# kobby-pentangeli/chaum-pedersen-zkp

Hardware: AMD Instinct MI355X
Metric: verified proofs/sec (1/2/4/8 MI355X) + % int-VALU roofline vs host-CPU (higher is better)
Workload: dtype int32/int64 limbs (GF(2^255-19), radix 2^25.5)

## Files before the change

### chaum-pedersen-zkp_amd/build_native.py

```python
from __future__ import annotations

import os
import shutil
import subprocess
import sys
from concurrent.futures import ThreadPoolExecutor

PKG = os.path.dirname(os.path.abspath(__file__))
ROOT = os.path.dirname(PKG)
CSRC = os.path.join(PKG, "csrc")
LIBDIR = os.path.join(PKG, "lib")
LIBCPZ = os.path.join(LIBDIR, "libcpz.so")
HOSTTEST = os.path.join(ROOT, "tests", "native", "libcpz_hosttest.so")
DEVPROBE = os.path.join(ROOT, "tests", "native", "libcpz_devprobe.so")
PARTPROBE = os.path.join(ROOT, "tests", "native", "libcpz_partprobe.so")
PARTPAIRSPROBE = os.path.join(ROOT, "tests", "native", "libcpz_partpairsprobe.so")
MSMPROBE = os.path.join(ROOT, "tests", "native", "libcpz_msmprobe.so")
PAIRSUMPROBE = os.path.join(ROOT, "tests", "native", "libcpz_pairsumprobe.so")
PREPPROBE = os.path.join(ROOT, "tests", "native", "libcpz_prepprobe.so")
MICROPROBE = os.path.join(ROOT, "tests", "native", "libcpz_microprobe.so")
ARCH = os.environ.get("CPZ_OFFLOAD_ARCH", "gfx950")


def _hipcc() -> str:
    for cand in (shutil.which("hipcc"), "/opt/rocm/bin/hipcc"):
        if cand and os.path.exists(cand):
            return cand
    raise RuntimeError("hipcc not found: the gfx950 build needs ROCm")


def _newer(out: str, srcs) -> bool:
    if not os.path.exists(out):
        return True
    t = os.path.getmtime(out)
    return any(os.path.getmtime(s) > t for s in srcs)


def _headers():
    hdr = [os.path.join(CSRC, f) for f in os.listdir(CSRC) if f.endswith(".h")]
    return hdr + [os.path.join(ROOT, "include", "cpz.h")]


def _run(cmd):
    r = subprocess.run(cmd, stdout=subprocess.PIPE, stderr=subprocess.STDOUT, text=True)
    if r.returncode != 0:
        raise RuntimeError("build step failed: %s\n%s" % (" ".join(cmd), r.stdout[-4000:]))
    return r.stdout


UNIT_FLAGS = {"wide.hip": ["-falign-loops=64"]}


def build_libcpz(force: bool = False, verbose: bool = False, out: str = LIBCPZ, defines=()) -> str:
    units = ["kernels.hip", "wide.hip", "rlc.hip", "part.hip", "runtime.hip"]
    srcs = [os.path.join(CSRC, u) for u in units] + _headers()
    if not force and not defines and not _newer(out, srcs):
        return out
    objdir = os.path.join(os.path.dirname(out), "obj" if not defines else "obj_" + "_".join(defines).replace("=", ""))
    os.makedirs(objdir, exist_ok=True)
    hipcc = _hipcc()
    common = [hipcc, "--offload-arch=" + ARCH, "-O3", "-std=c++17", "-fPIC", "-I", CSRC,
              "-I", os.path.join(ROOT, "include")] + ["-D" + d for d in defines]
    if defines and os.environ.get("CPZ_EXTRA_FLAGS"):
        common += os.environ["CPZ_EXTRA_FLAGS"].split()

    def compile_one(u):
        obj = os.path.join(objdir, u.replace(".hip", ".o"))
        if force or defines or _newer(obj, [os.path.join(CSRC, u)] + _headers()):
            uf = [] if defines and os.environ.get("CPZ_NO_UNIT_FLAGS") else UNIT_FLAGS.get(u, [])
            _run(common + uf + ["-c", os.path.join(CSRC, u), "-o", obj])
        return obj

    with ThreadPoolExecutor(max_workers=len(units)) as ex:
        objs = list(ex.map(compile_one, units))
    tmp = out + ".tmp"
    _run([hipcc, "--offload-arch=" + ARCH, "-shared", "-fPIC", "-o", tmp] + objs)
    os.replace(tmp, out)
    if verbose:
        print("built", out)
    return out


CLOCK_PROBE_LIB = os.path.join(LIBDIR, "timing", "clock_probe.so")


def build_clock_probe(force: bool = False) -> str:
    os.makedirs(os.path.dirname(CLOCK_PROBE_LIB), exist_ok=True)
    return build_libcpz(force, out=CLOCK_PROBE_LIB, defines=("CPZ_CLOCK_PROBE", "CPZ_TIMING_ONLY"))


def build_hosttest(force: bool = False, out: str = HOSTTEST, defines=()) -> str:
    srcs = [os.path.join(ROOT, "tests", "native", f) for f in ("hostlib.cpp", "hostlib_joint.cpp", "hostlib_lean.cpp",
                                                              "hostlib_prove.cpp", "hostlib_pairsum.cpp")]
    if not force and not _newer(out, srcs + _headers()):
        return out
    cxx = shutil.which("g++") or "g++"
    tmp = out + ".tmp"
    extra = ["-D" + d for d in os.environ.get("CPZ_HOST_DEFINES", "").split() + list(defines)]
    _run([cxx, "-O2", "-std=c++17", "-fPIC", "-shared", "-DCPZ_BOUNDS_CHECK", "-DCPZ_COUNT_OPS"] + extra +
         ["-I", CSRC] + srcs + ["-o", tmp])
    os.replace(tmp, out)
    return out


def build_devprobe(force: bool = False, out: str = DEVPROBE, include: str = CSRC) -> str:
    src = os.path.join(ROOT, "tests", "native", "devprobe.hip")
    hdrs = [os.path.join(include, f) for f in os.listdir(include) if f.endswith(".h")]
    if not force and not _newer(out, [src] + hdrs):
        return out
    tmp = out + ".tmp"
    _run([_hipcc(), "--offload-arch=" + ARCH, "-O3", "-std=c++17", "-fPIC", "-I", include,
          "-I", os.path.join(ROOT, "include"), "-shared", src, "-o", tmp])
    os.replace(tmp, out)
    return out


def build_partprobe(force: bool = False, out: str = PARTPROBE, include: str = CSRC) -> str:
    src = os.path.join(ROOT, "tests", "native", "partprobe.hip")
    deps = [os.path.join(include, f) for f in os.listdir(include) if f.endswith(".h") or f == "part.hip"]
    if not force and not _newer(out, [src] + deps):
        return out
    tmp = out + ".tmp"
    _run([_hipcc(), "--offload-arch=" + ARCH, "-O3", "-std=c++17", "-fPIC", "-I", include,
          "-I", os.path.join(ROOT, "include"), "-shared", src, "-o", tmp])
    os.replace(tmp, out)
    return out


def build_partpairsprobe(force: bool = False, out: str = PARTPAIRSPROBE, include: str = CSRC) -> str:
    src = os.path.join(ROOT, "tests", "native", "partpairsprobe.hip")
    deps = [os.path.join(include, f) for f in os.listdir(include) if f.endswith(".h") or f == "part.hip"]
    if not force and not _newer(out, [src] + deps):
        return out
    tmp = out + ".tmp"
    _run([_hipcc(), "--offload-arch=" + ARCH, "-O3", "-std=c++17", "-fPIC", "-I", include,
          "-I", os.path.join(ROOT, "include"), "-shared", src, "-o", tmp])
    os.replace(tmp, out)
    return out


def build_msmprobe(force: bool = False, out: str = MSMPROBE, include: str = CSRC) -> str:
    src = os.path.join(ROOT, "tests", "native", "msmprobe.hip")
    deps = [os.path.join(include, f) for f in os.listdir(include) if f.endswith(".h") or f == "rlc.hip"]
    if not force and not _newer(out, [src] + deps):
        return out
    tmp = out + ".tmp"
    _run([_hipcc(), "--offload-arch=" + ARCH, "-O3", "-std=c++17", "-fPIC", "-I", include,
          "-I", os.path.join(ROOT, "include"), "-shared", src, "-o", tmp])
    os.replace(tmp, out)
    return out


def build_pairsumprobe(force: bool = False, out: str = PAIRSUMPROBE, include: str = CSRC) -> str:
    src = os.path.join(ROOT, "tests", "native", "pairsumprobe.hip")
    deps = [os.path.join(include, f) for f in os.listdir(include) if f.endswith(".h") or f == "rlc.hip"]
    if not force and not _newer(out, [src] + deps):
        return out
    tmp = out + ".tmp"
    _run([_hipcc(), "--offload-arch=" + ARCH, "-O3", "-std=c++17", "-fPIC", "-I", include,
          "-I", os.path.join(ROOT, "include"), "-shared", src, "-o", tmp])
    os.replace(tmp, out)
    return out


def build_prepprobe(force: bool = False, out: str = PREPPROBE, include: str = CSRC) -> str:
    src = os.path.join(ROOT, "tests", "native", "prepprobe.hip")
    deps = [os.path.join(include, f) for f in os.listdir(include) if f.endswith(".h") or f == "rlc.hip"]
    if not force and not _newer(out, [src] + deps):
        return out
    tmp = out + ".tmp"
    _run([_hipcc(), "--offload-arch=" + ARCH, "-O3", "-std=c++17", "-fPIC", "-I", include,
          "-I", os.path.join(ROOT, "include"), "-shared", src, "-o", tmp])
    os.replace(tmp, out)
    return out


# ... 82 lines not shown
```

### chaum-pedersen-zkp_amd/csrc/fe25519.h

```cpp
#pragma once
#include <stdint.h>

#if defined(__HIPCC__)
#define CPZ_HD __host__ __device__ __forceinline__
#define CPZ_HDM __host__ __device__ __forceinline__
#else
#define CPZ_HD static inline
#define CPZ_HDM inline
#endif


#if defined(CPZ_BOUNDS_CHECK) && !defined(__HIP_DEVICE_COMPILE__)
#include <stdio.h>
#include <stdlib.h>
#define CPZ_ASSERT(c)                                                        \
  do {                                                                       \
    if (!(c)) {                                                              \
      fprintf(stderr, "cpz bound violated %s:%d: %s\n", __FILE__, __LINE__, #c); \
      abort();                                                               \
    }                                                                        \
  } while (0)
#else
#define CPZ_ASSERT(c) ((void)0)
#endif

namespace cpz {

#if defined(CPZ_COUNT_OPS) && !defined(__HIP_DEVICE_COMPILE__)
struct OpCounts {
  unsigned long long mul, sq;
};
inline OpCounts& op_counts() {
  static thread_local OpCounts c{0, 0};
  return c;
}
#define CPZ_COUNT(field) (++::cpz::op_counts().field)
#else
#define CPZ_COUNT(field) ((void)0)
#endif

struct fe {
  int32_t v[10];
};

constexpr int32_t kLooseBound = 108000000;

CPZ_HD fe fe_const(int32_t a0, int32_t a1, int32_t a2, int32_t a3, int32_t a4, int32_t a5,
                   int32_t a6, int32_t a7, int32_t a8, int32_t a9) {
  fe r;
  r.v[0] = a0; r.v[1] = a1; r.v[2] = a2; r.v[3] = a3; r.v[4] = a4;
  r.v[5] = a5; r.v[6] = a6; r.v[7] = a7; r.v[8] = a8; r.v[9] = a9;
  return r;
}

CPZ_HD fe fe_zero() { return fe_const(0, 0, 0, 0, 0, 0, 0, 0, 0, 0); }
CPZ_HD fe fe_one() { return fe_const(1, 0, 0, 0, 0, 0, 0, 0, 0, 0); }

CPZ_HD fe FE_D() { return fe_const(56195235, 13857412, 51736253, 6949390, 114729, 24766616, 60832955, 30306712, 48412415, 21499315); }
CPZ_HD fe FE_D2() { return fe_const(45281625, 27714825, 36363642, 13898781, 229458, 15978800, 54557047, 27058993, 29715967, 9444199); }
CPZ_HD fe FE_SQRT_M1() { return fe_const(34513072, 25610706, 9377949, 3500415, 12389472, 33281959, 41962654, 31548777, 326685, 11406482); }
CPZ_HD fe FE_INVSQRT_A_MINUS_D() { return fe_const(6111466, 4156064, 39310137, 12243467, 41204824, 120896, 20826367, 26493656, 6093567, 31568420); }
CPZ_HD fe FE_SQRT_AD_MINUS_ONE() { return fe_const(24849947, 33400850, 43495378, 6347714, 46036536, 32887293, 41837720, 18186727, 66238516, 14525638); }
CPZ_HD fe FE_ONE_MINUS_D_SQ() { return fe_const(6275446, 16937061, 44170319, 29780721, 11667076, 7397348, 39186143, 1766194, 42675006, 672202); }
CPZ_HD fe FE_INV2() { return fe_const(10, 0, 0, 0, 0, 0, 0, 0, 0, -16777216); }
CPZ_HD fe FE_D_MINUS_ONE_SQ() { return fe_const(15551776, 22456977, 53683765, 23429360, 55212328, 10178283, 40474537, 4729243, 61826754, 23438029); }

CPZ_HD fe fe_add(const fe& a, const fe& b) {
  fe r;
#pragma unroll
  for (int i = 0; i < 10; i++) r.v[i] = a.v[i] + b.v[i];
  return r;
}

CPZ_HD fe fe_sub(const fe& a, const fe& b) {
  fe r;
#pragma unroll
  for (int i = 0; i < 10; i++) r.v[i] = a.v[i] - b.v[i];
  return r;
}

CPZ_HD fe fe_neg(const fe& a) {
  fe r;
#pragma unroll
  for (int i = 0; i < 10; i++) r.v[i] = -a.v[i];
  return r;
}

CPZ_HD fe fe_select(const fe& a, const fe& b, bool c) {
  fe r;
#pragma unroll
  for (int i = 0; i < 10; i++) r.v[i] = c ? b.v[i] : a.v[i];
  return r;
}

#if defined(CPZ_BOUNDS_CHECK) && !defined(__HIP_DEVICE_COMPILE__)
CPZ_HD void fe_check_operand(const fe& a) {
  for (int i = 0; i < 10; i++) CPZ_ASSERT(a.v[i] < kLooseBound && a.v[i] > -kLooseBound);
}
#else
CPZ_HD void fe_check_operand(const fe&) {}
#endif

CPZ_HD constexpr int64_t carry_bias(int k) { return (k & 1) ? (1LL << 24) : (1LL << 25); }

CPZ_HD int64_t acc_pin(int64_t x) {
#if defined(__HIP_DEVICE_COMPILE__)
  asm("" : "+v"(x));
#endif
  return x;
}

CPZ_HD int32_t opaque_sgpr(int32_t x) {
#if defined(__HIP_DEVICE_COMPILE__)
  asm("" : "+s"(x));
#endif
  return x;
}

CPZ_HD int32_t unbias_limb(int64_t H, int k) {
  const uint32_t mask = (k & 1) ? 0x1ffffffu : 0x3ffffffu;
  return (int32_t)(((uint32_t)H & mask) - (uint32_t)carry_bias(k));
}

CPZ_HD fe fe_carry_biased(int64_t H[10]) {
  fe r;
  uint32_t small = 0;
#pragma unroll
  for (int k = 0; k < 9; k++) {
    const int w = (k & 1) ? 25 : 26;
    const int32_t hi = (int32_t)(H[k] >> 32);
    const uint32_t lo = (uint32_t)H[k];
    H[k + 1] = acc_pin((int64_t)hi * (int64_t)opaque_sgpr(1 << (32 - w)) + H[k + 1]);
    r.v[k] = (int32_t)((lo & ((1u << w) - 1u)) - (uint32_t)carry_bias(k) + small);
    small = lo >> w;
  }
  const int32_t hi9 = (int32_t)(H[9] >> 32);
  const uint32_t lo9 = (uint32_t)H[9];
  r.v[9] = (int32_t)((lo9 & 0x1ffffffu) - (uint32_t)carry_bias(9) + small);
  const int64_t h0 = (int64_t)hi9 * (int64_t)opaque_sgpr(19 << 7) +
                     (int64_t)(uint64_t)(((uint32_t)r.v[0] + (uint32_t)carry_bias(0)) + 19u * (lo9 >> 25));
  r.v[1] += (int32_t)(h0 >> 26);
  r.v[0] = unbias_limb(h0, 0);
  return r;
}

CPZ_HD fe fe_carry_wide(int64_t h[10]) {
#pragma unroll
  for (int k = 0; k < 10; k++) h[k] += carry_bias(k);
  return fe_carry_biased(h);
}

CPZ_HD fe fe_mul(const fe& f, const fe& g) {
  CPZ_COUNT(mul);
  fe_check_operand(f);
  fe_check_operand(g);
  int32_t g19[10], f2[10];
#pragma unroll
  for (int i = 0; i < 10; i++) {
    g19[i] = (int32_t)(19u * (uint32_t)g.v[i]);
    f2[i] = (int32_t)(2u * (uint32_t)f.v[i]);
  }
  int64_t h[10];
#pragma unroll
  for (int i = 0; i < 10; i++) {
#pragma unroll
    for (int k = 0; k < 10; k++) {
      const int j = (k - i + 10) % 10;
      const int32_t a = ((i & 1) && (j & 1)) ? f2[i] : f.v[i];
      const int32_t b = (i + j >= 10) ? g19[j] : g.v[j];
      h[k] = acc_pin((int64_t)a * (int64_t)b + (i == 0 ? carry_bias(k) : h[k]));
    }
  }
  fe r = fe_carry_biased(h);
  return r;
}

CPZ_HD void fe_sq_wide(int64_t h[10], const fe& f, int div) {
  CPZ_COUNT(sq);
  fe_check_operand(f);
  int32_t f2[10], f19[10];
#pragma unroll
  for (int i = 0; i < 10; i++) {
    f2[i] = (int32_t)(2u * (uint32_t)f.v[i]);
    f19[i] = (int32_t)(19u * (uint32_t)f.v[i]);
  }
  bool first[10] = {true, true, true, true, true, true, true, true, true, true};
#pragma unroll
  for (int i = 0; i < 10; i++) {
#pragma unroll
    for (int j = i; j < 10; j++) {
      const int k = (i + j) % 10;
      const int m2 = (i != j ? 2 : 1) * (((i & 1) && (j & 1)) ? 2 : 1);
      const int32_t a = (m2 == 1) ? f.v[i] : (m2 == 2 ? f2[i] : (int32_t)(2u * (uint32_t)f2[i]));
      const int32_t b = (i + j >= 10) ? f19[j] : f.v[j];
      h[k] = acc_pin((int64_t)a * (int64_t)b + (first[k] ? (div ? carry_bias(k) / div : 0) : h[k]));
      first[k] = false;
    }
  }
}

CPZ_HD fe fe_sq(const fe& f) {
  int64_t h[10];
  fe_sq_wide(h, f, 1);
  fe r = fe_carry_biased(h);
  return r;
}

CPZ_HD fe fe_sq2(const fe& f) {
  int64_t h[10];
  fe_sq_wide(h, f, 2);
#pragma unroll
  for (int i = 0; i < 10; i++) h[i] += h[i];
  fe r = fe_carry_biased(h);
  return r;
}

CPZ_HD fe fe_carry_floor(int64_t H[10]) {
  fe r;
#pragma unroll
  for (int k = 0; k < 9; k++) {
    H[k + 1] += H[k] >> ((k & 1) ? 25 : 26);
    r.v[k] = (int32_t)((uint32_t)H[k] & ((k & 1) ? 0x1ffffffu : 0x3ffffffu));
  }
  const int64_t h0 = (int64_t)r.v[0] + 19 * (H[9] >> 25);
  r.v[9] = (int32_t)((uint32_t)H[9] & 0x1ffffffu);
  r.v[1] += (int32_t)(h0 >> 26);
  r.v[0] = (int32_t)((uint32_t)h0 & 0x3ffffffu);
  return r;
}

CPZ_HD fe fe_sqn(fe f, int n) {
#pragma unroll 1
  for (int i = 1; i < n; i++) {
    int64_t h[10];
    fe_sq_wide(h, f, 0);
    f = fe_carry_floor(h);
  }
  return fe_sq(f);
}

CPZ_HD void fe_tobytes(uint8_t s[32], const fe& f) {
  int64_t h[10];
#pragma unroll
  for (int i = 0; i < 10; i++) h[i] = f.v[i];
  fe t = fe_carry_wide(h);
#pragma unroll
  for (int i = 0; i < 10; i++) h[i] = t.v[i];
  int64_t q = (19 * h[9] + (1 << 24)) >> 25;
  q = (h[0] + q) >> 26;
  q = (h[1] + q) >> 25;
  q = (h[2] + q) >> 26;
  q = (h[3] + q) >> 25;
  q = (h[4] + q) >> 26;
  q = (h[5] + q) >> 25;
  q = (h[6] + q) >> 26;
  q = (h[7] + q) >> 25;
  q = (h[8] + q) >> 26;
  q = (h[9] + q) >> 25;
  h[0] += 19 * q;
  int64_t c;
  c = h[0] >> 26; h[1] += c; h[0] -= c * (1LL << 26);
  c = h[1] >> 25; h[2] += c; h[1] -= c * (1LL << 25);
  c = h[2] >> 26; h[3] += c; h[2] -= c * (1LL << 26);
  c = h[3] >> 25; h[4] += c; h[3] -= c * (1LL << 25);
  c = h[4] >> 26; h[5] += c; h[4] -= c * (1LL << 26);
  c = h[5] >> 25; h[6] += c; h[5] -= c * (1LL << 25);
  c = h[6] >> 26; h[7] += c; h[6] -= c * (1LL << 26);
  c = h[7] >> 25; h[8] += c; h[7] -= c * (1LL << 25);
  c = h[8] >> 26; h[9] += c; h[8] -= c * (1LL << 26);
  c = h[9] >> 25; h[9] -= c * (1LL << 25);
  uint32_t w[8];
  const uint32_t l0 = (uint32_t)h[0], l1 = (uint32_t)h[1], l2 = (uint32_t)h[2], l3 = (uint32_t)h[3],
                 l4 = (uint32_t)h[4], l5 = (uint32_t)h[5], l6 = (uint32_t)h[6], l7 = (uint32_t)h[7],
                 l8 = (uint32_t)h[8], l9 = (uint32_t)h[9];
  w[0] = l0 | (l1 << 26);
  w[1] = (l1 >> 6) | (l2 << 19);
  w[2] = (l2 >> 13) | (l3 << 13);
  w[3] = (l3 >> 19) | (l4 << 6);
  w[4] = l5 | (l6 << 25);
  w[5] = (l6 >> 7) | (l7 << 19);
  w[6] = (l7 >> 13) | (l8 << 12);
  w[7] = (l8 >> 20) | (l9 << 6);
#pragma unroll
  for (int i = 0; i < 8; i++) {
    s[4 * i + 0] = (uint8_t)(w[i]);
    s[4 * i + 1] = (uint8_t)(w[i] >> 8);
    s[4 * i + 2] = (uint8_t)(w[i] >> 16);
    s[4 * i + 3] = (uint8_t)(w[i] >> 24);
  }
}

CPZ_HD void fe_towords(uint32_t w[8], const fe& f) {
  uint8_t s[32];
  fe_tobytes(s, f);
#pragma unroll
  for (int i = 0; i < 8; i++)
    w[i] = (uint32_t)s[4 * i] | ((uint32_t)s[4 * i + 1] << 8) | ((uint32_t)s[4 * i + 2] << 16) |
// ... 124 lines not shown
```

### chaum-pedersen-zkp_amd/csrc/kernels.hip

```cpp
#include <hip/hip_runtime.h>

#include <cstddef>
#include <type_traits>

#include "cpz_kernels.h"
#include "ristretto.h"
#include "scalar25519.h"
#include "transcript.h"
#include "scalarmul.h"
#include "verify.h"
#include "rlc_dev.h"
#include "fe16.h"
#include "keccak_wave.h"
#include "proof_digits.h"

namespace cpz {

__device__ __forceinline__ bool words_zero(const uint32_t w[8]) {
  uint32_t acc = 0;
#pragma unroll
  for (int k = 0; k < 8; k++) acc |= w[k];
  return acc == 0;
}

// ... 254 lines not shown
    if ((j >> bit) & 1) acc = ge_add(acc, Q);
  }
  comb[t] = p3_to_niels(acc);
}

__device__ __forceinline__ uint32_t be32_at(const uint8_t* p) {
  return ((uint32_t)p[0] << 24) | ((uint32_t)p[1] << 16) | ((uint32_t)p[2] << 8) | (uint32_t)p[3];
}

__device__ __forceinline__ void words_at(uint32_t w[8], const uint8_t* p) {
#pragma unroll
  for (int k = 0; k < 8; k++)
    w[k] = (uint32_t)p[4 * k] | ((uint32_t)p[4 * k + 1] << 8) | ((uint32_t)p[4 * k + 2] << 16) |
           ((uint32_t)p[4 * k + 3] << 24);
}

__global__ void __launch_bounds__(256) k_parse_proofs(ParseArgs a) {
  const int64_t i = (int64_t)blockIdx.x * 256 + threadIdx.x;
  if (i >= a.n) return;
  const uint64_t o0 = a.off[i];
  const uint64_t len = a.off[i + 1] - o0;
  const uint8_t* b = a.blob + o0;
  uint32_t f0[8], f1[8], f2[8];
#pragma unroll
  for (int k = 0; k < 8; k++) f0[k] = f1[k] = f2[k] = 0;
  uint8_t code = kParseOk;
  uint32_t aux = 0;
  if (len < 1 + 4 + 1 + 4 + 1 + 4 + 1) {
    code = kParseTooSmall;
    aux = (uint32_t)len;
  } else if (b[0] != 1) {
    code = kParseBadVersion;
    aux = b[0];
  } else {
    uint64_t pos = 1;
#pragma unroll 1
    for (int q = 0; q < 3 && code == kParseOk; q++) {
      const uint8_t base = (uint8_t)(kParseR1LenMissing + 5 * q);
      const uint32_t maxlen = q < 2 ? 4096u : 512u;
      if (pos + 4 > len) { code = base; break; }
      const uint32_t fl = be32_at(b + pos);
      pos += 4;
      if (fl == 0 || fl > maxlen) { code = base + 1; aux = fl; break; }
      if (pos + fl > len) { code = base + 2; break; }
      if (fl != 32) { code = base + 3; aux = fl; break; }
      uint32_t w[8];
      words_at(w, b + pos);
      pos += 32;
      bool ok;
      if (q < 2) {
        ge_p3 P;
        ok = ristretto_decode(P, w);
      } else {
        ok = sc_is_canonical(w);
      }
      if (!ok) { code = base + 4; break; }
#pragma unroll
      for (int k = 0; k < 8; k++) {
        f0[k] = q == 0 ? w[k] : f0[k];
        f1[k] = q == 1 ? w[k] : f1[k];
        f2[k] = q == 2 ? w[k] : f2[k];
      }
    }
    if (code == kParseOk && pos != len) {
      code = kParseTrailing;
      aux = (uint32_t)(len - pos);
    }
    if (code == kParseOk) {
      if (words_zero(f0) || words_zero(f1)) code = kParseIdentity;
      else if (words_zero(f2)) code = kParseZeroS;
    }
  }
  store_words8(a.r1, i, f0);
  store_words8(a.r2, i, f1);
  store_words8(a.s, i, f2);
  a.code[i] = code;
  if (a.aux) a.aux[i] = aux;
}


#ifndef CPZ_VERIFY_WAVES
#define CPZ_VERIFY_WAVES 2
#endif
__device__ __forceinline__ void verify_one_row(const VerifyArgs& a, int64_t i, const CombTable& comb_g,
                                               const CombTable& comb_h, const SlabTable& tab, uint32_t* dig,
                                               uint32_t* rows) {
  const uint32_t* src[4] = {a.y1, a.y2, a.r1, a.r2};
  uint32_t sw[8], cw[8];
#pragma unroll
  for (int q = 0; q < 4; q++) {
    uint32_t w[8];
    load_words8(w, src[q], i);
#pragma unroll
    for (int k = 0; k < 8; k++) rows[(8 * q + k) * kVerifyBlock] = w[k];
  }
  load_words8(sw, a.s, i);
  load_words8(cw, a.c, i);
  const uint8_t st_s = a.status[i];
  const DigitRef y1{rows, kVerifyBlock}, y2{rows + 8 * kVerifyBlock, kVerifyBlock},
      r1{rows + 16 * kVerifyBlock, kVerifyBlock}, r2{rows + 24 * kVerifyBlock, kVerifyBlock};
  a.status[i] = verify_proof(y1, y2, r1, r2, sw, cw, st_s, comb_g, comb_h, tab, dig, kVerifyBlock, nullptr,
                             a.eq_only != 0);
}

__global__ void __launch_bounds__(kVerifyBlock, CPZ_VERIFY_WAVES) k_verify_prepared(VerifyArgs a) {
  const CombTable comb_g{a.comb}, comb_h{a.comb + kCombPerBase};
  const int64_t l = (int64_t)blockIdx.x * kVerifyBlock + threadIdx.x;
  int64_t i = l;
  if (a.blocks) {
    const int64_t lb = (int64_t)blockIdx.x * (kVerifyBlock / a.block_proofs) + threadIdx.x / a.block_proofs;
    if (lb >= a.nblocks) return;
    i = (int64_t)a.blocks[lb] * a.block_proofs + threadIdx.x % a.block_proofs;
  }
  if (i >= a.n) return;
  const SlabTable tab{a.scratch, (uint32_t)l * (uint32_t)(kCachedEntries * sizeof(ge_cached))};
  __shared__ uint32_t dig[16 * kVerifyBlock];
  {
    if (a.status[i] != kStOk) return;
    uint32_t sw[8], cw[8];
    load_words8(sw, a.s, i);
    load_words8(cw, a.c, i);
    const DigitRef none{nullptr, 0};
    a.status[i] = verify_proof<true>(none, none, none, none, sw, cw, kStOk, comb_g, comb_h, tab, dig + threadIdx.x,
                                     kVerifyBlock, a.pre + 4 * i, a.eq_only != 0);
  }
}

__global__ void __launch_bounds__(kVerifyBlock, CPZ_VERIFY_WAVES) k_verify_each(VerifyArgs a) {
  const CombTable comb_g{a.comb}, comb_h{a.comb + kCombPerBase};
  const int64_t i = (int64_t)blockIdx.x * kVerifyBlock + threadIdx.x;
  if (i >= a.n) return;
#if defined(CPZ_EXP_SLAB_MOD)
  const SlabTable tab{a.scratch, (uint32_t)(i % CPZ_EXP_SLAB_MOD) * (uint32_t)(kCachedEntries * sizeof(ge_cached))};
#else
  const SlabTable tab{a.scratch, (uint32_t)i * (uint32_t)(kCachedEntries * sizeof(ge_cached))};
#endif
  __shared__ uint32_t dig[16 * kVerifyBlock];
  __shared__ uint32_t rows[32 * kVerifyBlock];
#if defined(CPZ_CLOCK_PROBE)
  const uint64_t t0 = __builtin_amdgcn_s_memtime(), q0 = __builtin_amdgcn_s_memrealtime();
#endif
  verify_one_row(a, i, comb_g, comb_h, tab, dig + threadIdx.x, rows + threadIdx.x);
#if defined(CPZ_CLOCK_PROBE)
  const uint64_t t1 = __builtin_amdgcn_s_memtime(), q1 = __builtin_amdgcn_s_memrealtime();
  if ((threadIdx.x & 63) == 0 && i + 63 < a.n) {
    uint32_t hw, xcc;
    asm volatile("s_getreg_b32 %0, hwreg(HW_REG_HW_ID)" : "=s"(hw));
    asm volatile("s_getreg_b32 %0, hwreg(HW_REG_XCC_ID)" : "=s"(xcc));
    uint64_t* out = reinterpret_cast<uint64_t*>(a.status + i);
    out[0] = t1 - t0;
    out[1] = q1 - q0;
    out[2] = q0;
    out[3] = q1;
    out[4] = (uint64_t)hw | ((uint64_t)xcc << 32);
  }
#endif
}

__device__ __forceinline__ sc chacha_scalar(const uint32_t key[8], uint64_t counter) {
  uint32_t blk[16];
  chacha20_block(blk, key, counter, 0);
  return sc_reduce_wide(blk);
}

__device__ __forceinline__ sc prove_scalar(const uint32_t* in, const uint32_t seed[8], uint64_t idx, int64_t i) {
  if (in == nullptr) return chacha_scalar(seed, idx);
  uint32_t wide[16];
  load_words8(wide, in, i);
#pragma unroll
  for (int k = 8; k < 16; k++) wide[k] = 0;
  return sc_reduce_wide(wide);
}

__global__ void __launch_bounds__(kVerifyBlock, 2) k_prove_points(ProveArgs a) {
  const CombTable comb_g{a.comb}, comb_h{a.comb + kCombPerBase};
  const int64_t i = (int64_t)blockIdx.x * kVerifyBlock + threadIdx.x;
  if (i >= a.n) return;
  const uint64_t idx = a.first_index + (uint64_t)i;
  uint32_t d[8], w[8];
  {
    const sc x = prove_scalar(a.x_in, a.seed_x, idx, i);
    sc_recode_radix65536(d, x.w);
  }
  ristretto_encode(w, comb_mul(comb_g, d));
  store_words8(a.y1, i, w);
  ristretto_encode(w, comb_mul(comb_h, d));
  store_words8(a.y2, i, w);
  {
    const sc k = prove_scalar(a.k_in, a.seed_k, idx, i);
    sc_recode_radix65536(d, k.w);
  }
  ristretto_encode(w, comb_mul(comb_g, d));
  store_words8(a.r1, i, w);
  ristretto_encode(w, comb_mul(comb_h, d));
  store_words8(a.r2, i, w);
}

__global__ void __launch_bounds__(kVerifyBlock, 2) k_prove_points_pairs(ProveArgs a, PairArgs pa) {
  const int64_t i = (int64_t)blockIdx.x * kVerifyBlock + threadIdx.x;
  if (i >= a.n) return;
  const uint64_t idx = a.first_index + (uint64_t)i;
  const ge_niels* tab = pa.desc[pa.pair_idx[i]].tab;
#pragma unroll 1
  for (int pass = 0; pass < 2; pass++) {
    uint32_t d[8], w[8];
    {
      const sc v = prove_scalar(pass ? a.k_in : a.x_in, pass ? a.seed_k : a.seed_x, idx, i);
      sc_recode_radix256(d, v.w);
    }
    ge_p3 G, H;
    pair_table_mul(G, H, tab, d);
#pragma unroll 1
    for (int e = 0; e < 2; e++) {
      ristretto_encode(w, G);
      G = H;
      store_words8(e ? (pass ? a.r2 : a.y2) : (pass ? a.r1 : a.y1), i, w);
    }
  }
}

__global__ void k_prove_response(ProveArgs a) {
// ... 754 lines not shown
```

### chaum-pedersen-zkp_amd/csrc/scalarmul.h

```cpp
#pragma once
#include "timing_only.h"
#include "ristretto.h"
#include "scalar25519.h"

#ifndef CPZ_LAZY_SIGN
#define CPZ_LAZY_SIGN 1
#endif
#ifndef CPZ_TABLE_LEAN
#define CPZ_TABLE_LEAN 1
#endif

namespace cpz {

constexpr int kTableV = 8;
constexpr int kTableSlots = kTableV + 1;
constexpr int kTableB = 128;

constexpr int kCombWindows = 16;
constexpr int kCombEntries = 1 << 15;
constexpr int kCombStride = kCombEntries + 1;
constexpr int64_t kCombPerBase = (int64_t)kCombWindows * kCombStride;

struct CombTable {
  const ge_niels* p;
// ... 131 lines not shown
#pragma unroll
    for (int t = 7; t > 0; t--) { cdig[t] = cdig[t - 1]; sdig[t] = sdig[t - 1]; }
#pragma unroll 1
    for (int m = 7; m >= 0; m--) {
      const int dc = ((int32_t)(wc << (28 - 4 * m))) >> 28;
      const ge_cached ev = cached_lookup(tab_v, dc);
      if (j != 7 || m != 7) cur = dbl4(cur);
      cur = ge_add_cached(p1p1_to_p3(cur), ev);
      if ((m & 1) == 0) {
        const int dg = ((int32_t)(wg << (24 - 8 * (m >> 1)))) >> 24;
        cur = ge_add_niels(p1p1_to_p3(cur), niels_lookup(tab_b, dg));
      }
    }
  }
  return p1p1_to_p3(cur);
}

template <class Comb, class Dig>
CPZ_HD ge_p1p1 comb_add(ge_p1p1 cur, const Comb& comb, const Dig& sd, int32_t sign = 0) {
#pragma unroll 1
  for (int j = 0; j < 8; j++) {
    const uint32_t w = sd[j];
#pragma unroll
    for (int m = 0; m < 2; m++) {
      const int d = (int32_t)(w << (16 - 16 * m)) >> 16;
#if CPZ_LAZY_SIGN
      const ge_niels e = comb_entry(comb, 2 * j + m, d < 0 ? -d : d, 0);
      cur = ge_add_niels(p1p1_to_p3(ge_p1p1_cneg(cur, d ^ sign)), e);
      sign = d;
#else
      cur = ge_add_niels(p1p1_to_p3(cur), comb.lookup(2 * j + m, d));
#endif
    }
  }
  return ge_p1p1_cneg(cur, sign);
}

constexpr int kJointSlots = 13;
CPZ_HD constexpr int joint_slot(int a, int b) { return 5 * a + b; }
CPZ_HD int joint_window(uint32_t wu, uint32_t wv, int m) { return joint_slot(radix4_digit(wu, m), radix4_digit(wv, m)); }
CPZ_HD int joint_top_window(uint32_t wu3, uint32_t wv3) {
  return joint_slot(radix4_top_digit(wu3), radix4_top_digit(wv3));
}

template <bool kFull = true>
CPZ_HD void build_joint_table(const SlabTable& tab, const ge_p3& Y, const ge_p3& R) {
  ge_niels nY, nR;
  nY.ypx = fe_add(Y.Y, Y.X);
  nY.ymx = fe_sub(Y.Y, Y.X);
  nY.xy2d = fe_mul(Y.T, FE_D2());
  nR.ypx = fe_add(R.Y, R.X);
  nR.ymx = fe_sub(R.Y, R.X);
  nR.xy2d = fe_mul(R.T, FE_D2());
  tab.store(0, ge_cached_identity());
  tab.store(joint_slot(1, 0), ge_cached{nY.ypx, nY.ymx, Y.Z, nY.xy2d});
  tab.store(joint_slot(0, 1), ge_cached{nR.ypx, nR.ymx, R.Z, nR.xy2d});
#pragma unroll 1
  for (int neg = 0; neg < 2; neg++) {
    const int s = neg ? -1 : 1;
    const ge_niels nRs = ge_niels_cneg(nR, neg != 0);
    ge_p3 A = Y;
#pragma unroll 1
    for (int j = 0; j < 3; j++) {
      const ge_p3 Q = p1p1_to_p3(ge_add_niels(A, j == 2 ? nY : nRs));
      tab.store(j == 0 ? joint_slot(1, s) : (j == 1 ? joint_slot(1, 2 * s) : joint_slot(2, s)), p3_to_cached(Q));
      if (j == 0) A = Q;
    }
    if constexpr (kFull) {
#pragma unroll 1
      for (int d = 0; d < 2; d++) {
        const ge_p3& P = d == 0 ? A : (neg ? R : Y);
        const int slot = d == 0 ? joint_slot(2, 2 * s) : (neg ? joint_slot(0, 2) : joint_slot(2, 0));
        tab.store(slot, p3_to_cached(p1p1_to_p3(p2_dbl(ge_p2{P.X, P.Y, P.Z}))));
      }
    } else {
      if (!neg) tab.store(joint_slot(2, 2), p3_to_cached(p1p1_to_p3(p2_dbl(ge_p2{A.X, A.Y, A.Z}))));
      const ge_p3& P = neg ? R : Y;
      const ge_p1p1 D = p2_dbl_zz2(P.X, P.Y, fe_add(fe_one(), fe_one()));
      tab.store(neg ? joint_slot(0, 2) : joint_slot(2, 0), p3_to_cached(p1p1_to_p3(D)));
    }
  }
}

CPZ_HD ge_p1p1 cached_to_p1p1(const ge_cached& e) {
  ge_p1p1 r;
  r.X = fe_sub(e.YpX, e.YmX);
  r.Y = fe_add(e.YpX, e.YmX);
  r.Z = fe_add(e.Z, e.Z);
  r.T = r.Z;
  return r;
}

template <class Comb, class Dig>
CPZ_HD ge_p1p1 straus_half_joint(const SlabTable& tab, const Comb& comb, const Dig& ud, const Dig& vd,
                                 const Dig& sdig) {
  ge_p1p1 cur = cached_to_p1p1(tab.load(joint_top_window(ud[3], vd[3])));
  int32_t sign = 0;
#pragma unroll 1
  for (int j = 3; j >= 0; j--) {
    const uint32_t wu = ud[j], wv = vd[j];
#pragma unroll 1
    for (int m = j == 3 ? 14 : 15; m >= 0; m--) {
      const int slot = joint_window(wu, wv, m);
#if CPZ_LAZY_SIGN
      const ge_cached e = tab.load(slot < 0 ? -slot : slot);
#else
      const ge_cached e = cached_lookup(tab, slot);
#endif
      cur = p2_dbl(p1p1_to_p2(cur));
      cur = p2_dbl(p1p1_to_p2(cur));
#if CPZ_LAZY_SIGN
      cur.X = fe_cneg(cur.X, slot ^ sign);
      sign = slot;
#endif
#if defined(CPZ_EXP_NIELS_TABLES)
      cur = ge_add_niels(p1p1_to_p3(cur), ge_niels{e.YpX, e.YmX, e.T2d, {0, 0}});
#else
      cur = ge_add_cached(p1p1_to_p3(cur), e);
#endif
    }
  }
  return comb_add(cur, comb, sdig, sign);
}

template <class Comb>
CPZ_HD ge_p3 comb_mul(const Comb& comb, const uint32_t sdig[8]) {
  return p1p1_to_p3(comb_add(p1p1_identity(), comb, host_digits(sdig)));
}

CPZ_HD ge_p3 fixed_base_mul(const ge_niels* tab_b, const uint32_t sdig_in[8]) {
  uint32_t sdig[8];
#pragma unroll
  for (int j = 0; j < 8; j++) sdig[j] = sdig_in[j];
  ge_p1p1 cur = p1p1_identity();
#pragma unroll 1
  for (int j = 7; j >= 0; j--) {
    const uint32_t wg = sdig[7];
#pragma unroll
    for (int t = 7; t > 0; t--) sdig[t] = sdig[t - 1];
#pragma unroll 1
    for (int m = 3; m >= 0; m--) {
      if (j != 7 || m != 3) {
        cur = dbl4(cur);
        cur = dbl4(cur);
      }
      const int dg = ((int32_t)(wg << (24 - 8 * m))) >> 24;
      cur = ge_add_niels(p1p1_to_p3(cur), niels_lookup(tab_b, dg));
    }
  }
  return p1p1_to_p3(cur);
}

constexpr int kNielsEntries = kTableB;
constexpr int kNielsLevelOfPart[8] = {0, 4, 2, 5, 1, 6, 3, 7};

CPZ_HD ge_niels niels_entry(const ge_niels* e) {
  ge_niels r;
#if defined(__HIP_DEVICE_COMPILE__)
  const uint4* s = reinterpret_cast<const uint4*>(e);
  uint4* d = reinterpret_cast<uint4*>(&r);
#pragma unroll
  for (int v = 0; v < (int)(sizeof(ge_niels) / 16); v++) d[v] = s[v];
#else
  r = *e;
#endif
  return r;
// ... 49 lines not shown
```

### chaum-pedersen-zkp_amd/csrc/verify.h

```cpp
#pragma once
#include "timing_only.h"
#include "ristretto.h"
#include "scalar25519.h"
#include "scalarmul.h"
#include "transcript.h"

#define CPZ_EQ_LOOP _Pragma("unroll 1")

namespace cpz {

constexpr uint8_t kStOk = 0, kStEqFail = 1, kStBadPoint = 2, kStBadScalar = 3, kStIdentity = 4, kStZeroS = 5;
constexpr uint8_t kStBadChallenge = 0x80;

CPZ_HD bool words8_zero(const uint32_t w[8]) {
  uint32_t acc = 0;
#pragma unroll
  for (int k = 0; k < 8; k++) acc |= w[k];
  return acc == 0;
}

CPZ_HD uint8_t response_status(const uint32_t s[8], bool eq_only = false) {
  if (!sc_is_canonical(s)) return kStBadScalar;
  if (sc_is_zero(s) && !eq_only) return kStZeroS;
  return kStOk;
// ... 102 lines not shown
    out[w] = (uint32_t)m[4 * w] | ((uint32_t)m[4 * w + 1] << 8) | ((uint32_t)m[4 * w + 2] << 16) |
             ((uint32_t)m[4 * w + 3] << 24);
}

CPZ_HD bool challenge_masks(uint32_t k1[50], uint32_t k2[50]) {
  MaskState ms;
  for (int g = 0; g < 3; g++)
    for (int i = 0; i < 200; i++) ms.m[g][i] = 0;
  Strobe<MaskState> s(ms, kTailPrefixPos, kTailPrefixBegin, (uint8_t)kTailPrefixFlags);
  const uint32_t z[8] = {0, 0, 0, 0, 0, 0, 0, 0};
  (void)transcript_challenge(s, z, z, z, z);
  if (ms.seg != 2) return false;
  for (int w = 0; w < 50; w++) {
    uint32_t a = 0, b = 0;
    for (int k = 3; k >= 0; k--) {
      a = (a << 8) | ms.m[0][4 * w + k];
      b = (b << 8) | ms.m[1][4 * w + k];
    }
    k1[w] = a;
    k2[w] = b;
  }
  return true;
}

template <class Acc>
CPZ_HD Strobe<Acc> transcript_new(Acc& st) {
  Strobe<Acc> s = strobe_init_merlin(st);
  s.merlin_header("dom-sep", 7, 25);
  s.absorb((const uint8_t*)"Chaum-Pedersen ZKP v1.0.0", 25);
  s.merlin_header("protocol", 8, 27);
  s.absorb((const uint8_t*)"chaum-pedersen-ristretto255", 27);
  return s;
}

template <class Acc>
CPZ_HD void transcript_context(Strobe<Acc>& s, const uint8_t* ctx, uint32_t len) {
  s.merlin_header("context", 7, len);
  for (uint32_t b = 0; b < len; b++) s.absorb_byte(ctx[b]);
}

template <class Acc>
CPZ_HD void transcript_parameters(Strobe<Acc>& s, const uint32_t g[8], const uint32_t h[8]) {
  s.merlin_append_words("generator-g", 11, g);
  s.merlin_append_words("generator-h", 11, h);
}

CPZ_HD bool challenge_masks_ctx32(uint32_t m[3][50], const uint32_t g[8], const uint32_t h[8]) {
  MaskState ms;
  for (int k = 0; k < 3; k++)
    for (int i = 0; i < 200; i++) ms.m[k][i] = 0;
  Strobe<MaskState> s(ms, kC32PrefixPos, kC32PrefixBegin, (uint8_t)kC32PrefixFlags);
  const uint8_t zc[32] = {0};
  const uint32_t z[8] = {0, 0, 0, 0, 0, 0, 0, 0};
  transcript_context(s, zc, 32);
  transcript_parameters(s, g, h);
  (void)transcript_challenge(s, z, z, z, z);
  if (ms.seg != 3) return false;
  for (int k = 0; k < 3; k++) mask_words(m[k], ms.m[k]);
  return true;
}

CPZ_HD ge_p3 affine_from_neg_niels(const ge_niels& q) {
  ge_p3 P;
  P.X = fe_mul(fe_sub(q.ymx, q.ypx), FE_INV2());
  P.Y = fe_mul(fe_add(q.ypx, q.ymx), FE_INV2());
  P.Z = fe_one();
  P.T = fe_mul(P.X, P.Y);
  return P;
}

CPZ_HD ge_niels niels_load(const ge_niels* p) {
  ge_niels r;
#if defined(__HIP_DEVICE_COMPILE__)
  const uint4* s = reinterpret_cast<const uint4*>(p);
  uint4* d = reinterpret_cast<uint4*>(&r);
#pragma unroll
  for (int v = 0; v < (int)(sizeof(ge_niels) / 16); v++) d[v] = s[v];
#else
  r = *p;
#endif
  return r;
}

template <bool kPre, class Comb, class Dig>
CPZ_HD bool check_equation(const Dig& y, const Dig& r, const ge_niels* pre_y, const ge_niels* pre_r,
                           const Dig& udig, const Dig& vdig, bool vneg, const Dig& sdig, const Comb& comb,
                           const SlabTable& tab, bool& decoded, bool& r_identity) {
  decoded = true;
  ge_p3 Yp, Rp;
CPZ_EQ_LOOP
  for (int k = 0; k < 2; k++) {
    ge_p3 P;
    if constexpr (kPre) {
      P = affine_from_neg_niels(niels_load(k ? pre_r : pre_y));
    } else {
      uint32_t w[8];
#pragma unroll
      for (int q = 0; q < 8; q++) w[q] = k ? r[q] : y[q];
      decoded = ristretto_decode(P, w) && decoded;
    }
    P = (k && vneg) ? P : ge_neg(P);
    if (k) Rp = P; else Yp = P;
  }
  build_joint_table<CPZ_TABLE_LEAN == 0>(tab, Yp, Rp);
  if constexpr (kPre) {
    r_identity = false;
  } else {
    uint32_t acc = 0;
#pragma unroll
    for (int q = 0; q < 8; q++) acc |= r[q];
    r_identity = acc == 0;
  }
#if defined(CPZ_EXP_EXTRA_INV)
  ge_p1p1 q = straus_half_joint(tab, comb, udig, vdig, sdig);
  q.X = fe_mul(q.X, fe_invert(q.Z));
  return ristretto_is_identity(q);
#else
  return ristretto_is_identity(straus_half_joint(tab, comb, udig, vdig, sdig));
#endif
}

template <bool kPre = false, class Comb>
CPZ_HD uint8_t verify_proof(const DigitRef& y1, const DigitRef& y2, const DigitRef& r1, const DigitRef& r2,
                            const uint32_t s[8], const uint32_t c[8], uint8_t st_s, const Comb& comb_g,
                            const Comb& comb_h, const SlabTable& tab_v, uint32_t* dig, int dstride,
                            const ge_niels* pre = nullptr, bool eq_only = false) {
  bool vneg;
#if defined(CPZ_EXP_NOSPLIT)
  vneg = c[7] & 1;
  for (int k = 0; k < 8; k++) {
    dig[k * dstride] = k % 4 == 3 ? c[k] & 0x3fffffffu : c[k];
    dig[(8 + k) * dstride] = s[k];
  }
  if (0)
#endif
  {
    uint32_t u[4], va[4], w[8];
    sc_half_split(c, u, va, vneg);
    sc_recode_radix4_half(w, u);
    sc_recode_radix4_half(w + 4, va);
    for (int k = 0; k < 8; k++) dig[k * dstride] = w[k];
    sc vs, ss;
#pragma unroll
    for (int k = 0; k < 8; k++) {
      vs.w[k] = k < 4 ? va[k] : 0u;
      ss.w[k] = s[k];
    }
    sc sp = sc_mul(vs, ss);
    if (vneg) sp = sc_neg(sp);
    sc_recode_radix65536(w, sp.w);
    for (int k = 0; k < 8; k++) dig[(8 + k) * dstride] = w[k];
  }
  const DigitRef udig{dig, dstride}, vdig{dig + 4 * dstride, dstride}, sdig{dig + 8 * dstride, dstride};
  bool dec = true, id = false, eq = true;
CPZ_EQ_LOOP
  for (int e = 0; e < 2; e++) {
    bool d, r_id;
    eq = check_equation<kPre>(e ? y2 : y1, e ? r2 : r1, kPre ? pre + 1 + 2 * e : nullptr, kPre ? pre + 2 * e : nullptr,
                              udig, vdig, vneg, sdig, e ? comb_h : comb_g, tab_v, d, r_id) && eq;
    dec = dec && d;
    id = id || r_id;
  }
  if (!dec) return kStBadPoint;
  if (st_s == kStBadScalar) return kStBadScalar;
  if (id && !eq_only) return kStIdentity;
  if (st_s == kStZeroS) return kStZeroS;
  if (st_s == kStBadChallenge) return kStBadScalar;
  return eq ? kStOk : kStEqFail;
}

}
```

Before: 56.15 million.

## Build joint table via LDS columns and fold sq2 doubling into multiplicands

Adds an LDS-backed joint-table build. Decoded Y/R points are written as cached fields into shared-memory columns, and each equation's proof rows are staged into LDS right before use. This is meant to cut register pressure during the table build. Separately, fe_sq2 now scales the multiplicands by 2 instead of computing a halved-bias square and doubling the 64-bit columns, which removes the extra adds. The trade-offs are more LDS traffic and a shared buffer that is larger than the row buffer it replaces, which may affect occupancy, plus more template plumbing.

```diff
diff --git a/chaum-pedersen-zkp_amd/build_native.py b/chaum-pedersen-zkp_amd/build_native.py
--- a/chaum-pedersen-zkp_amd/build_native.py
+++ b/chaum-pedersen-zkp_amd/build_native.py
@@ -91,7 +91,8 @@
 
 def build_hosttest(force: bool = False, out: str = HOSTTEST, defines=()) -> str:
     srcs = [os.path.join(ROOT, "tests", "native", f) for f in ("hostlib.cpp", "hostlib_joint.cpp", "hostlib_lean.cpp",
-                                                              "hostlib_prove.cpp", "hostlib_pairsum.cpp")]
+                                                              "hostlib_prove.cpp", "hostlib_pairsum.cpp",
+                                                              "hostlib_fold.cpp")]
     if not force and not _newer(out, srcs + _headers()):
         return out
     cxx = shutil.which("g++") or "g++"
diff --git a/chaum-pedersen-zkp_amd/csrc/fe25519.h b/chaum-pedersen-zkp_amd/csrc/fe25519.h
--- a/chaum-pedersen-zkp_amd/csrc/fe25519.h
+++ b/chaum-pedersen-zkp_amd/csrc/fe25519.h
@@ -24,6 +24,10 @@
 #define CPZ_ASSERT(c) ((void)0)
 #endif
 
+#ifndef CPZ_SQ2_FOLD
+#define CPZ_SQ2_FOLD 1
+#endif
+
 namespace cpz {
 
 #if defined(CPZ_COUNT_OPS) && !defined(__HIP_DEVICE_COMPILE__)
@@ -175,23 +179,26 @@
   return r;
 }
 
-CPZ_HD void fe_sq_wide(int64_t h[10], const fe& f, int div) {
+static_assert(8LL * kLooseBound < (1LL << 31), "8 f of a loose limb is a 32-bit multiplicand");
+static_assert(2.0 * 267.0 * (double)kLooseBound * (double)kLooseBound < 9.2e18, "doubled column below 2^63");
+
+template <int kScale>
+CPZ_HD void fe_sq_cols(int64_t h[10], const fe& f, int div) {
+  static_assert(kScale == 1 || kScale == 2, "the multiples of f are f, 2 f, 4 f, 8 f");
   CPZ_COUNT(sq);
   fe_check_operand(f);
-  int32_t f2[10], f19[10];
-#pragma unroll
-  for (int i = 0; i < 10; i++) {
-    f2[i] = (int32_t)(2u * (uint32_t)f.v[i]);
-    f19[i] = (int32_t)(19u * (uint32_t)f.v[i]);
-  }
+  int32_t f19[10];
+#pragma unroll
+  for (int i = 0; i < 10; i++) f19[i] = (int32_t)(19u * (uint32_t)f.v[i]);
   bool first[10] = {true, true, true, true, true, true, true, true, true, true};
 #pragma unroll
   for (int i = 0; i < 10; i++) {
 #pragma unroll
     for (int j = i; j < 10; j++) {
       const int k = (i + j) % 10;
-      const int m2 = (i != j ? 2 : 1) * (((i & 1) && (j & 1)) ? 2 : 1);
-      const int32_t a = (m2 == 1) ? f.v[i] : (m2 == 2 ? f2[i] : (int32_t)(2u * (uint32_t)f2[i]));
+      const int m = kScale * (i != j ? 2 : 1) * (((i & 1) && (j & 1)) ? 2 : 1);
+      const int32_t a = (int32_t)((uint32_t)m * (uint32_t)f.v[i]);
+      CPZ_ASSERT((int64_t)a == (int64_t)m * f.v[i]);
       const int32_t b = (i + j >= 10) ? f19[j] : f.v[j];
       h[k] = acc_pin((int64_t)a * (int64_t)b + (first[k] ? (div ? carry_bias(k) / div : 0) : h[k]));
       first[k] = false;
@@ -199,6 +206,8 @@
   }
 }
 
+CPZ_HD void fe_sq_wide(int64_t h[10], const fe& f, int div) { fe_sq_cols<1>(h, f, div); }
+
 CPZ_HD fe fe_sq(const fe& f) {
   int64_t h[10];
   fe_sq_wide(h, f, 1);
@@ -206,13 +215,28 @@
   return r;
 }
 
-CPZ_HD fe fe_sq2(const fe& f) {
+CPZ_HD fe fe_sq2_shift(const fe& f) {
   int64_t h[10];
   fe_sq_wide(h, f, 2);
 #pragma unroll
   for (int i = 0; i < 10; i++) h[i] += h[i];
   fe r = fe_carry_biased(h);
   return r;
+}
+
+CPZ_HD fe fe_sq2_fold(const fe& f) {
+  int64_t h[10];
+  fe_sq_cols<2>(h, f, 1);
+  fe r = fe_carry_biased(h);
+  return r;
+}
+
+CPZ_HD fe fe_sq2(const fe& f) {
+#if CPZ_SQ2_FOLD
+  return fe_sq2_fold(f);
+#else
+  return fe_sq2_shift(f);
+#endif
 }
 
 CPZ_HD fe fe_carry_floor(int64_t H[10]) {
diff --git a/chaum-pedersen-zkp_amd/csrc/kernels.hip b/chaum-pedersen-zkp_amd/csrc/kernels.hip
--- a/chaum-pedersen-zkp_amd/csrc/kernels.hip
+++ b/chaum-pedersen-zkp_amd/csrc/kernels.hip
@@ -360,11 +360,44 @@
 #ifndef CPZ_VERIFY_WAVES
 #define CPZ_VERIFY_WAVES 2
 #endif
+#ifndef CPZ_BUILD_LDS
+#define CPZ_BUILD_LDS 1
+#endif
+static_assert(!CPZ_BUILD_LDS || CPZ_TABLE_LEAN, "the LDS build is the lean one");
+constexpr int kVerifyRowWords = CPZ_BUILD_LDS ? kBuildWords : 32;
+constexpr int kStageY = 0, kStageR = kBuildWords - 8;
+static_assert((16 + kVerifyRowWords) * kVerifyBlock * 4 <= 80 * 1024, "two k_verify_each blocks per CU");
+
+#if CPZ_BUILD_LDS
+struct StageRows {
+  const VerifyArgs& a;
+  int64_t i;
+  uint32_t* rows;
+  __device__ __forceinline__ void operator()(int e) const {
+    uint32_t w[8];
+    load_words8(w, e ? a.y2 : a.y1, i);
+#pragma unroll
+    for (int k = 0; k < 8; k++) rows[(kStageY + k) * kVerifyBlock] = w[k];
+    load_words8(w, e ? a.r2 : a.r1, i);
+#pragma unroll
+    for (int k = 0; k < 8; k++) rows[(kStageR + k) * kVerifyBlock] = w[k];
+  }
+};
+#endif
+
 __device__ __forceinline__ void verify_one_row(const VerifyArgs& a, int64_t i, const CombTable& comb_g,
                                                const CombTable& comb_h, const SlabTable& tab, uint32_t* dig,
                                                uint32_t* rows) {
+  uint32_t sw[8], cw[8];
+#if CPZ_BUILD_LDS
+  load_words8(sw, a.s, i);
+  load_words8(cw, a.c, i);
+  const uint8_t st_s = a.status[i];
+  const DigitRef y{rows + kStageY * kVerifyBlock, kVerifyBlock}, r{rows + kStageR * kVerifyBlock, kVerifyBlock};
+  a.status[i] = verify_proof(y, y, r, r, sw, cw, st_s, comb_g, comb_h, tab, dig, kVerifyBlock, nullptr,
+                             a.eq_only != 0, BuildCols{rows, kVerifyBlock}, StageRows{a, i, rows});
+#else
   const uint32_t* src[4] = {a.y1, a.y2, a.r1, a.r2};
-  uint32_t sw[8], cw[8];
 #pragma unroll
   for (int q = 0; q < 4; q++) {
     uint32_t w[8];
@@ -379,6 +412,7 @@
       r1{rows + 16 * kVerifyBlock, kVerifyBlock}, r2{rows + 24 * kVerifyBlock, kVerifyBlock};
   a.status[i] = verify_proof(y1, y2, r1, r2, sw, cw, st_s, comb_g, comb_h, tab, dig, kVerifyBlock, nullptr,
                              a.eq_only != 0);
+#endif
 }
 
 __global__ void __launch_bounds__(kVerifyBlock, CPZ_VERIFY_WAVES) k_verify_prepared(VerifyArgs a) {
@@ -399,8 +433,15 @@
     load_words8(sw, a.s, i);
     load_words8(cw, a.c, i);
     const DigitRef none{nullptr, 0};
+#if CPZ_BUILD_LDS
+    __shared__ uint32_t bld[kBuildWords * kVerifyBlock];
+    a.status[i] = verify_proof<true>(none, none, none, none, sw, cw, kStOk, comb_g, comb_h, tab, dig + threadIdx.x,
+                                     kVerifyBlock, a.pre + 4 * i, a.eq_only != 0,
+                                     BuildCols{bld + threadIdx.x, kVerifyBlock});
+#else
     a.status[i] = verify_proof<true>(none, none, none, none, sw, cw, kStOk, comb_g, comb_h, tab, dig + threadIdx.x,
                                      kVerifyBlock, a.pre + 4 * i, a.eq_only != 0);
+#endif
   }
 }
 
@@ -414,7 +455,7 @@
   const SlabTable tab{a.scratch, (uint32_t)i * (uint32_t)(kCachedEntries * sizeof(ge_cached))};
 #endif
   __shared__ uint32_t dig[16 * kVerifyBlock];
-  __shared__ uint32_t rows[32 * kVerifyBlock];
+  __shared__ uint32_t rows[kVerifyRowWords * kVerifyBlock];
 #if defined(CPZ_CLOCK_PROBE)
   const uint64_t t0 = __builtin_amdgcn_s_memtime(), q0 = __builtin_amdgcn_s_memrealtime();
 #endif
diff --git a/chaum-pedersen-zkp_amd/csrc/scalarmul.h b/chaum-pedersen-zkp_amd/csrc/scalarmul.h
--- a/chaum-pedersen-zkp_amd/csrc/scalarmul.h
+++ b/chaum-pedersen-zkp_amd/csrc/scalarmul.h
@@ -237,6 +237,76 @@
   }
 }
 
+constexpr int kBuildFields = 6;
+constexpr int kBuildWords = 10 * kBuildFields;
+struct BuildCols {
+  uint32_t* p;
+  int stride;
+  CPZ_HDM fe load(int f) const {
+    const uint32_t* q = p + 10 * f * stride;
+    fe r;
+#pragma unroll
+    for (int k = 0; k < 10; k++) r.v[k] = (int32_t)q[k * stride];
+    return r;
+  }
+  CPZ_HDM void store(int f, const fe& x) const {
+    uint32_t* q = p + 10 * f * stride;
+#pragma unroll
+    for (int k = 0; k < 10; k++) q[k * stride] = (uint32_t)x.v[k];
+  }
+  CPZ_HDM void affine(int f0, fe& X, fe& Y) const {
+    const fe ypx = load(f0), ymx = load(f0 + 1);
+#pragma unroll
+    for (int k = 0; k < 10; k++) {
+      X.v[k] = (ypx.v[k] - ymx.v[k]) >> 1;
+      Y.v[k] = (ypx.v[k] + ymx.v[k]) >> 1;
+    }
+  }
+  CPZ_HDM void put_point(int which, const ge_p3& P, const SlabTable& tab) const {
+    ge_cached c;
+    c.YpX = fe_add(P.Y, P.X);
+    c.YmX = fe_sub(P.Y, P.X);
+    c.Z = P.Z;
+    c.T2d = fe_mul(P.T, FE_D2());
+    store(3 * which, c.YpX);
+    store(3 * which + 1, c.YmX);
+    store(3 * which + 2, c.T2d);
+    tab.store(which ? joint_slot(0, 1) : joint_slot(1, 0), c);
+  }
+};
+
+CPZ_HD void build_joint_table_cols(const SlabTable& tab, const BuildCols& cols, const fe& YT) {
+#pragma unroll 1
+  for (int neg = 0; neg < 2; neg++) {
+    const int s = neg ? -1 : 1;
+    ge_p3 A;
+    cols.affine(0, A.X, A.Y);
+    A.Z = fe_one();
+    A.T = YT;
+#pragma unroll 1
+    for (int j = 0; j < 3; j++) {
+      const int f0 = j == 2 ? 0 : 3, swap = j == 2 ? 0 : neg;
+      const fe PP = fe_mul(fe_add(A.Y, A.X), cols.load(f0 + swap));
+      const fe MM = fe_mul(fe_sub(A.Y, A.X), cols.load(f0 + 1 - swap));
+      const fe Txy2d = fe_mul(A.T, fe_cneg(cols.load(f0 + 2), -swap));
+      const fe Z2 = fe_add(A.Z, A.Z);
+      ge_p1p1 r;
+      r.X = fe_sub(PP, MM);
+      r.Y = fe_add(PP, MM);
+      r.Z = fe_add(Z2, Txy2d);
+      r.T = fe_sub(Z2, Txy2d);
+      const ge_p3 Q = p1p1_to_p3(r);
+      tab.store(j == 0 ? joint_slot(1, s) : (j == 1 ? joint_slot(1, 2 * s) : joint_slot(2, s)), p3_to_cached(Q));
+      if (j == 0) A = Q;
+    }
+    if (!neg) tab.store(joint_slot(2, 2), p3_to_cached(p1p1_to_p3(p2_dbl(ge_p2{A.X, A.Y, A.Z}))));
+    fe PX, PY;
+    cols.affine(neg ? 3 : 0, PX, PY);
+    const ge_p1p1 D = p2_dbl_zz2(PX, PY, fe_add(fe_one(), fe_one()));
+    tab.store(neg ? joint_slot(0, 2) : joint_slot(2, 0), p3_to_cached(p1p1_to_p3(D)));
+  }
+}
+
 CPZ_HD ge_p1p1 cached_to_p1p1(const ge_cached& e) {
   ge_p1p1 r;
   r.X = fe_sub(e.YpX, e.YmX);
diff --git a/chaum-pedersen-zkp_amd/csrc/verify.h b/chaum-pedersen-zkp_amd/csrc/verify.h
--- a/chaum-pedersen-zkp_amd/csrc/verify.h
+++ b/chaum-pedersen-zkp_amd/csrc/verify.h
@@ -208,34 +208,59 @@
   return r;
 }
 
-template <bool kPre, class Comb, class Dig>
+struct BuildInRegs {};
+template <class Build> struct build_in_cols { static constexpr bool value = false; };
+template <> struct build_in_cols<BuildCols> { static constexpr bool value = true; };
+
+template <bool kPre, class Comb, class Dig, class Build>
 CPZ_HD bool check_equation(const Dig& y, const Dig& r, const ge_niels* pre_y, const ge_niels* pre_r,
                            const Dig& udig, const Dig& vdig, bool vneg, const Dig& sdig, const Comb& comb,
-                           const SlabTable& tab, bool& decoded, bool& r_identity) {
+                           const SlabTable& tab, bool& decoded, bool& r_identity, const Build& build) {
   decoded = true;
-  ge_p3 Yp, Rp;
+  r_identity = false;
+  if constexpr (build_in_cols<Build>::value) {
+    fe YT = fe_zero();
 CPZ_EQ_LOOP
-  for (int k = 0; k < 2; k++) {
-    ge_p3 P;
-    if constexpr (kPre) {
-      P = affine_from_neg_niels(niels_load(k ? pre_r : pre_y));
-    } else {
-      uint32_t w[8];
-#pragma unroll
-      for (int q = 0; q < 8; q++) w[q] = k ? r[q] : y[q];
-      decoded = ristretto_decode(P, w) && decoded;
-    }
-    P = (k && vneg) ? P : ge_neg(P);
-    if (k) Rp = P; else Yp = P;
-  }
-  build_joint_table<CPZ_TABLE_LEAN == 0>(tab, Yp, Rp);
-  if constexpr (kPre) {
-    r_identity = false;
+    for (int k = 0; k < 2; k++) {
+      const bool is_r = k == 0;
+      ge_p3 P;
+      if constexpr (kPre) {
+        P = affine_from_neg_niels(niels_load(is_r ? pre_r : pre_y));
+      } else {
+        uint32_t w[8];
+#pragma unroll
+        for (int q = 0; q < 8; q++) w[q] = is_r ? r[q] : y[q];
+        if (is_r) r_identity = words8_zero(w);
+        decoded = ristretto_decode(P, w) && decoded;
+      }
+      P = (is_r && vneg) ? P : ge_neg(P);
+      build.put_point(is_r ? 1 : 0, P, tab);
+      YT = P.T;
+    }
+    build_joint_table_cols(tab, build, YT);
   } else {
-    uint32_t acc = 0;
-#pragma unroll
-    for (int q = 0; q < 8; q++) acc |= r[q];
-    r_identity = acc == 0;
+    ge_p3 Yp, Rp;
+CPZ_EQ_LOOP
+    for (int k = 0; k < 2; k++) {
+      ge_p3 P;
+      if constexpr (kPre) {
+        P = affine_from_neg_niels(niels_load(k ? pre_r : pre_y));
+      } else {
+        uint32_t w[8];
+#pragma unroll
+        for (int q = 0; q < 8; q++) w[q] = k ? r[q] : y[q];
+        decoded = ristretto_decode(P, w) && decoded;
+      }
+      P = (k && vneg) ? P : ge_neg(P);
+      if (k) Rp = P; else Yp = P;
+    }
+    build_joint_table<CPZ_TABLE_LEAN == 0>(tab, Yp, Rp);
+    if constexpr (!kPre) {
+      uint32_t acc = 0;
+#pragma unroll
+      for (int q = 0; q < 8; q++) acc |= r[q];
+      r_identity = acc == 0;
+    }
   }
 #if defined(CPZ_EXP_EXTRA_INV)
   ge_p1p1 q = straus_half_joint(tab, comb, udig, vdig, sdig);
@@ -246,11 +271,16 @@
 #endif
 }
 
-template <bool kPre = false, class Comb>
+struct StageNothing {
+  CPZ_HDM void operator()(int) const {}
+};
+
+template <bool kPre = false, class Comb, class Build = BuildInRegs, class Stage = StageNothing>
 CPZ_HD uint8_t verify_proof(const DigitRef& y1, const DigitRef& y2, const DigitRef& r1, const DigitRef& r2,
                             const uint32_t s[8], const uint32_t c[8], uint8_t st_s, const Comb& comb_g,
                             const Comb& comb_h, const SlabTable& tab_v, uint32_t* dig, int dstride,
-                            const ge_niels* pre = nullptr, bool eq_only = false) {
+                            const ge_niels* pre = nullptr, bool eq_only = false, const Build& build = Build(),
+                            const Stage& stage = Stage()) {
   bool vneg;
 #if defined(CPZ_EXP_NOSPLIT)
   vneg = c[7] & 1;
@@ -279,11 +309,13 @@
   }
   const DigitRef udig{dig, dstride}, vdig{dig + 4 * dstride, dstride}, sdig{dig + 8 * dstride, dstride};
   bool dec = true, id = false, eq = true;
+  if constexpr (build_in_cols<Build>::value) tab_v.store(0, ge_cached_identity());
 CPZ_EQ_LOOP
   for (int e = 0; e < 2; e++) {
     bool d, r_id;
+    stage(e);
     eq = check_equation<kPre>(e ? y2 : y1, e ? r2 : r1, kPre ? pre + 1 + 2 * e : nullptr, kPre ? pre + 2 * e : nullptr,
-                              udig, vdig, vneg, sdig, e ? comb_h : comb_g, tab_v, d, r_id) && eq;
+                              udig, vdig, vneg, sdig, e ? comb_h : comb_g, tab_v, d, r_id, build) && eq;
     dec = dec && d;
     id = id || r_id;
   }
```

New measurement: 56.71 million, median of 6. +1.0%, better.
